# graphdeco-inria/hierarchical-3d-gaussians

Measured on NVIDIA H100. Metric: train-step images/sec (fwd+bwd) @1080p, 3M Gaussians, SH-3, higher is better.
Workload: dtype f32

## Files before the change

### hierarchical-3d-gaussians_b200/csrc/preprocess_backward.cu

```cuda
#include "common.cuh"
#include "cov_grad.cuh"

namespace h3dgs {

__device__ __constant__ float bSH_C2[5] = {1.0925484305920792f, -1.0925484305920792f, 0.31539156525252005f,
                                           -1.0925484305920792f, 0.5462742152960396f};
__device__ __constant__ float bSH_C3[7] = {-0.5900435899266435f, 2.890611442640554f, -0.4570457994644658f,
                                           0.3731763325901154f, -0.4570457994644658f, 1.445305721320277f,
                                           -0.5900435899266435f};
constexpr float bSH_C0 = 0.28209479177387814f;
constexpr float bSH_C1 = 0.4886025119029199f;

__device__ __forceinline__ void store_zero(float* p, int n) {
    for (int k = 0; k < n; k++) p[k] = 0.f;
}

__global__ void __launch_bounds__(128)
preprocess_backward_kernel(int row0, int P, const RowCycle cyc, int deg, int M, const float* __restrict__ means3D, const float* __restrict__ scales,
                           float scale_mod, const float* __restrict__ rots, const float* __restrict__ shs,
                           const float* __restrict__ cov3D_precomp, const float* __restrict__ colors_precomp,
                           const float* __restrict__ ts, const int* __restrict__ ridx, const int* __restrict__ pidx,
                           const float* __restrict__ view, const float* __restrict__ proj,
                           const float* __restrict__ campos, int W, int H, float tanx, float tany, float fx, float fy,
                           int use_depth, const int* __restrict__ radii, const uint8_t* __restrict__ rank_mask, const StagePtrs peers,
                           const Record* __restrict__ records,
                           const float* __restrict__ accum, float* __restrict__ dL_dmeans3D,
                           float* __restrict__ dL_dmeans2D, float* __restrict__ dL_dsh, float* __restrict__ dL_dcolors,
                           float* __restrict__ dL_dopacities, float* __restrict__ dL_dscales,
                           float* __restrict__ dL_drots, float* __restrict__ dL_dcov3D)
{
    __shared__ float s_view[16], s_proj[16];
    if (threadIdx.x < 16) { s_view[threadIdx.x] = view[threadIdx.x]; s_proj[threadIdx.x] = proj[threadIdx.x]; }
    __syncthreads();
    const int local = blockIdx.x * blockDim.x + threadIdx.x;
    const int i = cyc.world > 1 ? cyclic_row(cyc, local) : row0 + local;
    if (i >= P) return;

    if (radii[i] <= 0) {
        store_zero(dL_dmeans2D + 3 * i, 3);
        if (ridx) return;
        store_zero(dL_dmeans3D + 3 * i, 3);
        dL_dopacities[i] = 0.f;
        if (dL_dcolors) store_zero(dL_dcolors + 3 * i, 3);
        if (dL_dscales) store_zero(dL_dscales + 3 * i, 3);
        if (dL_drots) store_zero(dL_drots + 4 * i, 4);
        if (dL_dcov3D) store_zero(dL_dcov3D + 6 * i, 6);
        return;
    }

    const float* v = s_view;
    float ac[kAccum];
    if (peers.n > 1) gather_accum_pairs<5>(peers, rank_mask[i], i, 0, ac);
    else {
        const float2* row = reinterpret_cast<const float2*>(accum + (size_t)i * kAccum);
#pragma unroll
        for (int k = 0; k < 5; k++) { const float2 v = row[k]; ac[2 * k] = v.x; ac[2 * k + 1] = v.y; }
    }
    const float g_mx = ac[0] * (0.5f * W), g_my = ac[1] * (0.5f * H);
    const float dcx = -0.5f * ac[2], dcy = -0.5f * ac[3], dcz = -0.5f * ac[4], g_op = ac[5];
    const float g_r = ac[6], g_g = ac[7], g_b = ac[8], g_iv = ac[9];
    int c = i, p = i;
    float t = 1.0f, u = 0.0f;
    if (ridx) {
        c = ridx[i]; p = pidx[i]; if (p < 0) p = c;
        t = ts[i]; u = 1.0f - t;
    }
    const bool lerp = ridx != nullptr && u != 0.0f;
#define LERP(a, b) (lerp ? __fadd_rn(__fmul_rn(t, (a)), __fmul_rn(u, (b))) : (a))
    const float mx = LERP(means3D[3 * c], means3D[3 * p]);
    const float my = LERP(means3D[3 * c + 1], means3D[3 * p + 1]);
    const float mz = LERP(means3D[3 * c + 2], means3D[3 * p + 2]);
    float qsign = 1.0f;

    float cov6[6], R[3][3], Mm[3][3], sc[3], qv[4] = {1.f, 0.f, 0.f, 0.f};
    const bool have_sr = cov3D_precomp == nullptr;
    if (!have_sr) {
#pragma unroll
        for (int k = 0; k < 6; k++) cov6[k] = cov3D_precomp[6 * c + k];
    } else {
        float4 qq = *reinterpret_cast<const float4*>(rots + 4 * c);
        if (lerp) {
            float4 qp = *reinterpret_cast<const float4*>(rots + 4 * p);
            const float dot = __fadd_rn(__fadd_rn(__fadd_rn(__fmul_rn(qq.x, qp.x), __fmul_rn(qq.y, qp.y)), __fmul_rn(qq.z, qp.z)), __fmul_rn(qq.w, qp.w));
            if (dot < 0.f) qsign = -1.0f;
            qq.x = LERP(qq.x, qsign * qp.x); qq.y = LERP(qq.y, qsign * qp.y);
            qq.z = LERP(qq.z, qsign * qp.z); qq.w = LERP(qq.w, qsign * qp.w);
        }
        qv[0] = qq.x; qv[1] = qq.y; qv[2] = qq.z; qv[3] = qq.w;
#pragma unroll
        for (int k = 0; k < 3; k++) sc[k] = scale_mod * LERP(scales[3 * c + k], scales[3 * p + k]);
        cov3d_from_scale_quat(sc, qv, R, Mm, cov6);
    }

    CovGradOut cg;
    cov_chain_backward(v, mx, my, mz, fx, fy, tanx, tany, kFovClamp, kDilation, cov6, dcx, dcy, dcz, g_iv, use_depth != 0,
                       have_sr, sc, qv, R, Mm, scale_mod, cg);
    float dmean[3] = {cg.dmean[0], cg.dmean[1], cg.dmean[2]};
    {
        const float* q = s_proj;
        const float hw = q[3] * mx + q[7] * my + q[11] * mz + q[15];
        const float m_w = 1.0f / (hw + kWEps);
        const float mul1 = (q[0] * mx + q[4] * my + q[8] * mz + q[12]) * m_w * m_w;
        const float mul2 = (q[1] * mx + q[5] * my + q[9] * mz + q[13]) * m_w * m_w;
        dmean[0] += (q[0] * m_w - q[3] * mul1) * g_mx + (q[1] * m_w - q[3] * mul2) * g_my;
        dmean[1] += (q[4] * m_w - q[7] * mul1) * g_mx + (q[5] * m_w - q[7] * mul2) * g_my;
        dmean[2] += (q[8] * m_w - q[11] * mul1) * g_mx + (q[9] * m_w - q[11] * mul2) * g_my;
    }
    dL_dmeans2D[3 * i] = g_mx; dL_dmeans2D[3 * i + 1] = g_my; dL_dmeans2D[3 * i + 2] = 0.f;
#define EMIT(ptr, width, k, val)                                                           \
    do {                                                                                   \
        const float v__ = (val);                                                           \
        if (!ridx) (ptr)[(size_t)i * (width) + (k)] = v__;                                 \
        else {                                                                             \
            atomicAdd((ptr) + (size_t)c * (width) + (k), t * v__);                         \
            if (lerp) atomicAdd((ptr) + (size_t)p * (width) + (k), u * v__);               \
        }                                                                                  \
    } while (0)
    EMIT(dL_dopacities, 1, 0, g_op);

    if (colors_precomp && dL_dcolors) { dL_dcolors[3 * c] = g_r; dL_dcolors[3 * c + 1] = g_g; dL_dcolors[3 * c + 2] = g_b; }
    EMIT(dL_dmeans3D, 3, 0, dmean[0]); EMIT(dL_dmeans3D, 3, 1, dmean[1]); EMIT(dL_dmeans3D, 3, 2, dmean[2]);

    if (!have_sr) {
        if (dL_dcov3D) {
#pragma unroll
            for (int k = 0; k < 6; k++) dL_dcov3D[6 * c + k] = cg.g6[k];
        }
    } else {
#pragma unroll
        for (int k = 0; k < 3; k++) EMIT(dL_dscales, 3, k, cg.dscale[k]);
        const float4 dq = make_float4(cg.dq[0], cg.dq[1], cg.dq[2], cg.dq[3]);
        if (!ridx) *reinterpret_cast<float4*>(dL_drots + 4 * i) = dq;
        else {
            atomicAdd(reinterpret_cast<float4*>(dL_drots) + c, make_float4(t * dq.x, t * dq.y, t * dq.z, t * dq.w));
            if (lerp) {
                const float us = u * qsign;
                atomicAdd(reinterpret_cast<float4*>(dL_drots) + p, make_float4(us * dq.x, us * dq.y, us * dq.z, us * dq.w));
            }
        }
    }
#undef EMIT
#undef LERP
}

__global__ void __launch_bounds__(128)
sh_backward_kernel(int row0, int P, const RowCycle cyc, int deg, int M, const float* __restrict__ means3D, const float* __restrict__ shs,
                   const float* __restrict__ ts, const int* __restrict__ ridx, const int* __restrict__ pidx,
                   const float* __restrict__ campos, const int* __restrict__ radii, const uint8_t* __restrict__ rank_mask,
                   const StagePtrs peers, const Record* __restrict__ records,
                   const float* __restrict__ accum, float* __restrict__ dL_dmeans3D, float* __restrict__ dL_dsh)
{
    const int local = blockIdx.x * blockDim.x + threadIdx.x;
    const int i = cyc.world > 1 ? cyclic_row(cyc, local) : row0 + local;
    if (i >= P) return;
    const int SH3 = M * 3;
    if (radii[i] <= 0) {
        if (!ridx) {
            float* o = dL_dsh + (size_t)i * SH3;
            if ((SH3 & 3) == 0) { for (int k = 0; k < SH3 / 4; k++) reinterpret_cast<float4*>(o)[k] = make_float4(0, 0, 0, 0); }
            else store_zero(o, SH3);
        }
        return;
    }
    int c = i, p = i;
    float t = 1.0f, u = 0.0f;
    if (ridx) {
        c = ridx[i]; p = pidx[i]; if (p < 0) p = c;
        t = ts[i]; u = 1.0f - t;
    }
    const bool lerp = ridx != nullptr && u != 0.0f;
#define LERP(a, b) (lerp ? __fadd_rn(__fmul_rn(t, (a)), __fmul_rn(u, (b))) : (a))
    const float mx = LERP(means3D[3 * c], means3D[3 * p]);
    const float my = LERP(means3D[3 * c + 1], means3D[3 * p + 1]);
    const float mz = LERP(means3D[3 * c + 2], means3D[3 * p + 2]);
    float col[4];
    if (peers.n > 1) gather_accum_pairs<2>(peers, rank_mask[i], i, 3, col);
    else { const float* ac = accum + (size_t)i * kAccum; col[0] = ac[6]; col[1] = ac[7]; col[2] = ac[8]; }
    const uint32_t kb = __float_as_uint(records[i].b.w);
    const float dRGB[3] = {(kb >> kClampShift) & 1u ? 0.f : col[0], (kb >> (kClampShift + 1)) & 1u ? 0.f : col[1],
                           (kb >> (kClampShift + 2)) & 1u ? 0.f : col[2]};
    const float d0x = mx - campos[0], d0y = my - campos[1], d0z = mz - campos[2];
    const float len = sqrtf(d0x * d0x + d0y * d0y + d0z * d0z);
    const float x = d0x / len, y = d0y / len, z = d0z / len;
    const int ncoef = (deg + 1) * (deg + 1);
    float B[16], Bx[16], By[16], Bz[16];
#pragma unroll
    for (int k = 0; k < 16; k++) { B[k] = 0.f; Bx[k] = 0.f; By[k] = 0.f; Bz[k] = 0.f; }
    B[0] = bSH_C0;
    if (deg > 0) {
        B[1] = -bSH_C1 * y; B[2] = bSH_C1 * z; B[3] = -bSH_C1 * x;
        By[1] = -bSH_C1; Bz[2] = bSH_C1; Bx[3] = -bSH_C1;
        if (deg > 1) {
            const float xx = x * x, yy = y * y, zz = z * z, xy = x * y, yz = y * z, xz = x * z;
            B[4] = bSH_C2[0] * xy; B[5] = bSH_C2[1] * yz; B[6] = bSH_C2[2] * (2.f * zz - xx - yy);
            B[7] = bSH_C2[3] * xz; B[8] = bSH_C2[4] * (xx - yy);
            Bx[4] = bSH_C2[0] * y; By[4] = bSH_C2[0] * x;
            By[5] = bSH_C2[1] * z; Bz[5] = bSH_C2[1] * y;
            Bx[6] = bSH_C2[2] * 2.f * -x; By[6] = bSH_C2[2] * 2.f * -y; Bz[6] = bSH_C2[2] * 2.f * 2.f * z;
            Bx[7] = bSH_C2[3] * z; Bz[7] = bSH_C2[3] * x;
            Bx[8] = bSH_C2[4] * 2.f * x; By[8] = bSH_C2[4] * 2.f * -y;
            if (deg > 2) {
                B[9] = bSH_C3[0] * y * (3.f * xx - yy); B[10] = bSH_C3[1] * xy * z;
                B[11] = bSH_C3[2] * y * (4.f * zz - xx - yy); B[12] = bSH_C3[3] * z * (2.f * zz - 3.f * xx - 3.f * yy);
                B[13] = bSH_C3[4] * x * (4.f * zz - xx - yy); B[14] = bSH_C3[5] * z * (xx - yy);
                B[15] = bSH_C3[6] * x * (xx - 3.f * yy);
                Bx[9] = bSH_C3[0] * 3.f * 2.f * xy;   By[9] = bSH_C3[0] * 3.f * (xx - yy);
                Bx[10] = bSH_C3[1] * yz;              By[10] = bSH_C3[1] * xz;               Bz[10] = bSH_C3[1] * xy;
                Bx[11] = bSH_C3[2] * -2.f * xy;       By[11] = bSH_C3[2] * (-3.f * yy + 4.f * zz - xx); Bz[11] = bSH_C3[2] * 4.f * 2.f * yz;
                Bx[12] = bSH_C3[3] * -3.f * 2.f * xz; By[12] = bSH_C3[3] * -3.f * 2.f * yz;  Bz[12] = bSH_C3[3] * 3.f * (2.f * zz - xx - yy);
                Bx[13] = bSH_C3[4] * (-3.f * xx + 4.f * zz - yy); By[13] = bSH_C3[4] * -2.f * xy; Bz[13] = bSH_C3[4] * 4.f * 2.f * xz;
                Bx[14] = bSH_C3[5] * 2.f * xz;        By[14] = bSH_C3[5] * -2.f * yz;        Bz[14] = bSH_C3[5] * (xx - yy);
                Bx[15] = bSH_C3[6] * 3.f * (xx - yy); By[15] = bSH_C3[6] * -3.f * 2.f * xy;
            }
        }
    }
    float ddx = 0.f, ddy = 0.f, ddz = 0.f;
    const float* shc = shs + (size_t)c * SH3;
    const float* shp = shs + (size_t)p * SH3;
    float* dshi = dL_dsh + (size_t)i * SH3;
    if ((SH3 & 3) == 0) {
#pragma unroll
        for (int q = 0; q < 12; q++) {
            if (4 * q < SH3) {
                float o4[4] = {0.f, 0.f, 0.f, 0.f};
                if (4 * q < 3 * ncoef) {
                    float4 v = __ldg(reinterpret_cast<const float4*>(shc) + q);
                    if (lerp) {
                        const float4 w = __ldg(reinterpret_cast<const float4*>(shp) + q);
                        v.x = LERP(v.x, w.x); v.y = LERP(v.y, w.y); v.z = LERP(v.z, w.z); v.w = LERP(v.w, w.w);
                    }
                    const float sv[4] = {v.x, v.y, v.z, v.w};
#pragma unroll
                    for (int r = 0; r < 4; r++) {
                        const int e = 4 * q + r, k = e / 3, ch = e - 3 * k;
                        const float g = dRGB[ch];
                        o4[r] = B[k] * g;
                        ddx += Bx[k] * sv[r] * g; ddy += By[k] * sv[r] * g; ddz += Bz[k] * sv[r] * g;
                    }
                }
                if (!ridx) reinterpret_cast<float4*>(dshi)[q] = make_float4(o4[0], o4[1], o4[2], o4[3]);
                else if (4 * q < 3 * ncoef) {
                    atomicAdd(reinterpret_cast<float4*>(dL_dsh + (size_t)c * SH3) + q, make_float4(t * o4[0], t * o4[1], t * o4[2], t * o4[3]));
                    if (lerp) atomicAdd(reinterpret_cast<float4*>(dL_dsh + (size_t)p * SH3) + q, make_float4(u * o4[0], u * o4[1], u * o4[2], u * o4[3]));
                }
            }
        }
    } else {
#pragma unroll
        for (int e = 0; e < 48; e++) {
            if (e < SH3) {
                const int k = e / 3, ch = e - 3 * k;
                float o = 0.f;
                if (e < 3 * ncoef) {
                    const float sv = LERP(__ldg(shc + e), __ldg(shp + e));
                    const float g = dRGB[ch];
                    o = B[k] * g;
                    ddx += Bx[k] * sv * g; ddy += By[k] * sv * g; ddz += Bz[k] * sv * g;
                }
                if (!ridx) dshi[e] = o;
                else if (e < 3 * ncoef) {
                    atomicAdd(dL_dsh + (size_t)c * SH3 + e, t * o);
                    if (lerp) atomicAdd(dL_dsh + (size_t)p * SH3 + e, u * o);
                }
            }
        }
    }
    const float sum2 = d0x * d0x + d0y * d0y + d0z * d0z;
    const float invsum32 = 1.0f / sqrtf(sum2 * sum2 * sum2);
    const float dm0 = ((sum2 - d0x * d0x) * ddx - d0y * d0x * ddy - d0z * d0x * ddz) * invsum32;
    const float dm1 = (-d0x * d0y * ddx + (sum2 - d0y * d0y) * ddy - d0z * d0y * ddz) * invsum32;
    const float dm2 = (-d0x * d0z * ddx - d0y * d0z * ddy + (sum2 - d0z * d0z) * ddz) * invsum32;
    if (!ridx) {
        dL_dmeans3D[3 * i] += dm0; dL_dmeans3D[3 * i + 1] += dm1; dL_dmeans3D[3 * i + 2] += dm2;
    } else {
        atomicAdd(dL_dmeans3D + 3 * (size_t)c + 0, t * dm0); atomicAdd(dL_dmeans3D + 3 * (size_t)c + 1, t * dm1);
        atomicAdd(dL_dmeans3D + 3 * (size_t)c + 2, t * dm2);
        if (lerp) {
            atomicAdd(dL_dmeans3D + 3 * (size_t)p + 0, u * dm0); atomicAdd(dL_dmeans3D + 3 * (size_t)p + 1, u * dm1);
            atomicAdd(dL_dmeans3D + 3 * (size_t)p + 2, u * dm2);
        }
    }
#undef LERP
}

__global__ void __launch_bounds__(256)
peer_push_kernel(int P, const RowCycle cyc, const uint8_t* __restrict__ rank_mask, const float* __restrict__ accum,
                 const PeerPtrs stages)
{
    const int i = blockIdx.x * blockDim.x + threadIdx.x;
    if (i >= P) return;
    if (!((rank_mask[i] >> cyc.rank) & 1u)) return;
    const int owner = (i >> cyc.shift) % cyc.world;
    if (owner == cyc.rank) return;
    float* dst = nullptr;
#pragma unroll
    for (int r = 0; r < H3DGS_MAX_PEERS; r++) if (r == owner) dst = static_cast<float*>(stages.p[r]);
    float2* d2 = reinterpret_cast<float2*>(dst + ((size_t)cyc.rank * P + i) * kAccum);
    const float2* s2 = reinterpret_cast<const float2*>(accum + (size_t)i * kAccum);
#pragma unroll
    for (int k = 0; k < kAccum / 2; k++) d2[k] = s2[k];
}

int launch_peer_push(const h3dgs_raster_args& a, const uint8_t* rank_mask, const float* accum, cudaStream_t s)
{
    if (a.P == 0 || a.peer_count <= 1) return H3DGS_OK;
    const RowCycle cyc = row_cycle(a);
    peer_push_kernel<<<(a.P + 255) / 256, 256, 0, s>>>(a.P, cyc, rank_mask, accum, peer_ptrs(a.peer_stage, a.peer_count));
    H3_LAUNCHED("peer_push", a.debug, s);
    return H3DGS_OK;
}

int launch_preprocess_backward(const h3dgs_raster_args& a, const int32_t* radii, const uint8_t* rank_mask, const Record* records,
                               const float* accum, float* dL_dmeans3D, float* dL_dmeans2D, float* dL_dsh,
                               float* dL_dcolors, float* dL_dopacities, float* dL_dscales, float* dL_drots,
                               float* dL_dcov3D, cudaStream_t s)
{
    if (a.P == 0) return H3DGS_OK;
    const float fx = a.image_width / (2.0f * a.tanfovx), fy = a.image_height / (2.0f * a.tanfovy);
    const RowCycle cyc = row_cycle(a);
    const int r0 = (cyc.world > 1 || a.grad_row_end <= a.grad_row_begin) ? 0 : a.grad_row_begin;
    const int r1 = (cyc.world > 1 || a.grad_row_end <= a.grad_row_begin) ? a.P : min(a.grad_row_end, a.P);
    const int rows = cyc.world > 1 ? cyclic_local_rows(cyc, a.P) : r1 - r0;
    if (rows <= 0) return H3DGS_OK;
    ProfScope prof(H3DGS_STAGE_PREPROCESS_BWD, s);
    preprocess_backward_kernel<<<(rows + 127) / 128, 128, 0, s>>>(
        r0, r1, cyc, a.sh_degree, a.sh_coeffs, a.means3D, a.scales, a.scale_modifier, a.rotations, a.shs, a.cov3D_precomp,
        a.colors_precomp, a.interpolation_weights, a.render_indices, a.parent_indices, a.viewmatrix, a.projmatrix, a.campos, a.image_width, a.image_height, a.tanfovx, a.tanfovy,
        fx, fy, a.do_depth, radii, rank_mask, stage_ptrs(a, accum), records, accum, dL_dmeans3D, dL_dmeans2D, dL_dsh, dL_dcolors, dL_dopacities,
        dL_dscales, dL_drots, dL_dcov3D);
    H3_LAUNCHED("preprocess_backward", a.debug, s);
    return H3DGS_OK;
}

int launch_sh_backward(const h3dgs_raster_args& a, const int32_t* radii, const uint8_t* rank_mask, const Record* records,
                       const float* accum, float* dL_dmeans3D, float* dL_dsh, cudaStream_t s)
{
    if (a.P == 0 || a.colors_precomp) return H3DGS_OK;
    const RowCycle cyc = row_cycle(a);
    const int r0 = (cyc.world > 1 || a.grad_row_end <= a.grad_row_begin) ? 0 : a.grad_row_begin;
    const int r1 = (cyc.world > 1 || a.grad_row_end <= a.grad_row_begin) ? a.P : min(a.grad_row_end, a.P);
    const int rows = cyc.world > 1 ? cyclic_local_rows(cyc, a.P) : r1 - r0;
    if (rows <= 0) return H3DGS_OK;
    ProfScope prof(H3DGS_STAGE_SH_BACKWARD, s);
    sh_backward_kernel<<<(rows + 127) / 128, 128, 0, s>>>(r0, r1, cyc, a.sh_degree, a.sh_coeffs, a.means3D, a.shs,
                                                         a.interpolation_weights, a.render_indices, a.parent_indices,
                                                         a.campos, radii, rank_mask, stage_ptrs(a, accum), records, accum,
                                                         dL_dmeans3D, dL_dsh);
    H3_LAUNCHED("sh_backward", a.debug, s);
    return H3DGS_OK;
}

}
```

Baseline: 317.9.

## Stage SH rows through shared memory for coalesced loads and stores in SH backward

Adds a templated SH backward kernel in which each warp cooperatively loads the SH coefficient rows of its 32 Gaussians into padded shared memory with coalesced float4 reads, computes per-thread gradients from shared memory, then writes dL_dsh back cooperatively. This replaces the per-thread strided 192-byte row accesses, which coalesce poorly, and factors the SH basis computation into a shared helper. The cost is about 26KB of shared memory per 128-thread block at degree 3, which may limit occupancy.

```diff
diff --git a/hierarchical-3d-gaussians_b200/csrc/preprocess_backward.cu b/hierarchical-3d-gaussians_b200/csrc/preprocess_backward.cu
--- a/hierarchical-3d-gaussians_b200/csrc/preprocess_backward.cu
+++ b/hierarchical-3d-gaussians_b200/csrc/preprocess_backward.cu
@@ -143,47 +143,9 @@
 #undef LERP
 }
 
-__global__ void __launch_bounds__(128)
-sh_backward_kernel(int row0, int P, const RowCycle cyc, int deg, int M, const float* __restrict__ means3D, const float* __restrict__ shs,
-                   const float* __restrict__ ts, const int* __restrict__ ridx, const int* __restrict__ pidx,
-                   const float* __restrict__ campos, const int* __restrict__ radii, const uint8_t* __restrict__ rank_mask,
-                   const StagePtrs peers, const Record* __restrict__ records,
-                   const float* __restrict__ accum, float* __restrict__ dL_dmeans3D, float* __restrict__ dL_dsh)
-{
-    const int local = blockIdx.x * blockDim.x + threadIdx.x;
-    const int i = cyc.world > 1 ? cyclic_row(cyc, local) : row0 + local;
-    if (i >= P) return;
-    const int SH3 = M * 3;
-    if (radii[i] <= 0) {
-        if (!ridx) {
-            float* o = dL_dsh + (size_t)i * SH3;
-            if ((SH3 & 3) == 0) { for (int k = 0; k < SH3 / 4; k++) reinterpret_cast<float4*>(o)[k] = make_float4(0, 0, 0, 0); }
-            else store_zero(o, SH3);
-        }
-        return;
-    }
-    int c = i, p = i;
-    float t = 1.0f, u = 0.0f;
-    if (ridx) {
-        c = ridx[i]; p = pidx[i]; if (p < 0) p = c;
-        t = ts[i]; u = 1.0f - t;
-    }
-    const bool lerp = ridx != nullptr && u != 0.0f;
-#define LERP(a, b) (lerp ? __fadd_rn(__fmul_rn(t, (a)), __fmul_rn(u, (b))) : (a))
-    const float mx = LERP(means3D[3 * c], means3D[3 * p]);
-    const float my = LERP(means3D[3 * c + 1], means3D[3 * p + 1]);
-    const float mz = LERP(means3D[3 * c + 2], means3D[3 * p + 2]);
-    float col[4];
-    if (peers.n > 1) gather_accum_pairs<2>(peers, rank_mask[i], i, 3, col);
-    else { const float* ac = accum + (size_t)i * kAccum; col[0] = ac[6]; col[1] = ac[7]; col[2] = ac[8]; }
-    const uint32_t kb = __float_as_uint(records[i].b.w);
-    const float dRGB[3] = {(kb >> kClampShift) & 1u ? 0.f : col[0], (kb >> (kClampShift + 1)) & 1u ? 0.f : col[1],
-                           (kb >> (kClampShift + 2)) & 1u ? 0.f : col[2]};
-    const float d0x = mx - campos[0], d0y = my - campos[1], d0z = mz - campos[2];
-    const float len = sqrtf(d0x * d0x + d0y * d0y + d0z * d0z);
-    const float x = d0x / len, y = d0y / len, z = d0z / len;
-    const int ncoef = (deg + 1) * (deg + 1);
-    float B[16], Bx[16], By[16], Bz[16];
+__device__ __forceinline__ void sh_basis(int deg, float x, float y, float z, float (&B)[16], float (&Bx)[16], float (&By)[16],
+                                         float (&Bz)[16])
+{
 #pragma unroll
     for (int k = 0; k < 16; k++) { B[k] = 0.f; Bx[k] = 0.f; By[k] = 0.f; Bz[k] = 0.f; }
     B[0] = bSH_C0;
@@ -214,6 +176,50 @@
             }
         }
     }
+}
+
+__global__ void __launch_bounds__(128)
+sh_backward_kernel(int row0, int P, const RowCycle cyc, int deg, int M, const float* __restrict__ means3D, const float* __restrict__ shs,
+                   const float* __restrict__ ts, const int* __restrict__ ridx, const int* __restrict__ pidx,
+                   const float* __restrict__ campos, const int* __restrict__ radii, const uint8_t* __restrict__ rank_mask,
+                   const StagePtrs peers, const Record* __restrict__ records,
+                   const float* __restrict__ accum, float* __restrict__ dL_dmeans3D, float* __restrict__ dL_dsh)
+{
+    const int local = blockIdx.x * blockDim.x + threadIdx.x;
+    const int i = cyc.world > 1 ? cyclic_row(cyc, local) : row0 + local;
+    if (i >= P) return;
+    const int SH3 = M * 3;
+    if (radii[i] <= 0) {
+        if (!ridx) {
+            float* o = dL_dsh + (size_t)i * SH3;
+            if ((SH3 & 3) == 0) { for (int k = 0; k < SH3 / 4; k++) reinterpret_cast<float4*>(o)[k] = make_float4(0, 0, 0, 0); }
+            else store_zero(o, SH3);
+        }
+        return;
+    }
+    int c = i, p = i;
+    float t = 1.0f, u = 0.0f;
+    if (ridx) {
+        c = ridx[i]; p = pidx[i]; if (p < 0) p = c;
+        t = ts[i]; u = 1.0f - t;
+    }
+    const bool lerp = ridx != nullptr && u != 0.0f;
+#define LERP(a, b) (lerp ? __fadd_rn(__fmul_rn(t, (a)), __fmul_rn(u, (b))) : (a))
+    const float mx = LERP(means3D[3 * c], means3D[3 * p]);
+    const float my = LERP(means3D[3 * c + 1], means3D[3 * p + 1]);
+    const float mz = LERP(means3D[3 * c + 2], means3D[3 * p + 2]);
+    float col[4];
+    if (peers.n > 1) gather_accum_pairs<2>(peers, rank_mask[i], i, 3, col);
+    else { const float* ac = accum + (size_t)i * kAccum; col[0] = ac[6]; col[1] = ac[7]; col[2] = ac[8]; }
+    const uint32_t kb = __float_as_uint(records[i].b.w);
+    const float dRGB[3] = {(kb >> kClampShift) & 1u ? 0.f : col[0], (kb >> (kClampShift + 1)) & 1u ? 0.f : col[1],
+                           (kb >> (kClampShift + 2)) & 1u ? 0.f : col[2]};
+    const float d0x = mx - campos[0], d0y = my - campos[1], d0z = mz - campos[2];
+    const float len = sqrtf(d0x * d0x + d0y * d0y + d0z * d0z);
+    const float x = d0x / len, y = d0y / len, z = d0z / len;
+    const int ncoef = (deg + 1) * (deg + 1);
+    float B[16], Bx[16], By[16], Bz[16];
+    sh_basis(deg, x, y, z, B, Bx, By, Bz);
     float ddx = 0.f, ddy = 0.f, ddz = 0.f;
     const float* shc = shs + (size_t)c * SH3;
     const float* shp = shs + (size_t)p * SH3;
@@ -283,6 +289,121 @@
 #undef LERP
 }
 
+template <int Q>
+__global__ void __launch_bounds__(128)
+sh_backward_rows_kernel(int row0, int P, const RowCycle cyc, int deg, const float* __restrict__ means3D, const float* __restrict__ shs,
+                        const float* __restrict__ ts, const int* __restrict__ ridx, const int* __restrict__ pidx,
+                        const float* __restrict__ campos, const int* __restrict__ radii, const uint8_t* __restrict__ rank_mask,
+                        const StagePtrs peers, const Record* __restrict__ records,
+                        const float* __restrict__ accum, float* __restrict__ dL_dmeans3D, float* __restrict__ dL_dsh)
+{
+    constexpr int SH3 = 4 * Q;
+    constexpr int kStride = SH3 + 4;
+    __shared__ __align__(16) float s_row[128 * kStride];
+    __shared__ int s_c[128], s_p[128];
+    __shared__ float s_t[128], s_u[128];
+    const int tid = threadIdx.x, lane = tid & 31, wb = tid - lane;
+    const int local = blockIdx.x * blockDim.x + threadIdx.x;
+    const int i = cyc.world > 1 ? cyclic_row(cyc, local) : row0 + local;
+    const bool live = i < P && radii[i] > 0;
+    int c = i, p = i;
+    float t = 1.0f, u = 0.0f;
+    if (live && ridx) {
+        c = ridx[i]; p = pidx[i]; if (p < 0) p = c;
+        t = ts[i]; u = 1.0f - t;
+    }
+    const bool lerp = live && ridx != nullptr && u != 0.0f;
+    if (i < P && !live && !ridx) {
+#pragma unroll
+        for (int q = 0; q < Q; q++) reinterpret_cast<float4*>(dL_dsh + (size_t)i * SH3)[q] = make_float4(0.f, 0.f, 0.f, 0.f);
+    }
+    s_c[tid] = live ? c : -1; s_p[tid] = lerp ? p : -1; s_t[tid] = t; s_u[tid] = u;
+    __syncwarp();
+    for (int k = lane; k < 32 * Q; k += 32) {
+        const int r = wb + k / Q, q = k % Q;
+        const int cr = s_c[r];
+        if (cr < 0) continue;
+        float4 v = __ldg(reinterpret_cast<const float4*>(shs + (size_t)cr * SH3) + q);
+        const int pr = s_p[r];
+        if (pr >= 0) {
+            const float4 w = __ldg(reinterpret_cast<const float4*>(shs + (size_t)pr * SH3) + q);
+            const float tr = s_t[r], ur = s_u[r];
+            v.x = __fadd_rn(__fmul_rn(tr, v.x), __fmul_rn(ur, w.x)); v.y = __fadd_rn(__fmul_rn(tr, v.y), __fmul_rn(ur, w.y));
+            v.z = __fadd_rn(__fmul_rn(tr, v.z), __fmul_rn(ur, w.z)); v.w = __fadd_rn(__fmul_rn(tr, v.w), __fmul_rn(ur, w.w));
+        }
+        reinterpret_cast<float4*>(s_row + r * kStride)[q] = v;
+    }
+    __syncwarp();
+    const int ncoef = (deg + 1) * (deg + 1);
+    if (live) {
+#define LERP(a, b) (lerp ? __fadd_rn(__fmul_rn(t, (a)), __fmul_rn(u, (b))) : (a))
+        const float mx = LERP(means3D[3 * c], means3D[3 * p]);
+        const float my = LERP(means3D[3 * c + 1], means3D[3 * p + 1]);
+        const float mz = LERP(means3D[3 * c + 2], means3D[3 * p + 2]);
+#undef LERP
+        float col[4];
+        if (peers.n > 1) gather_accum_pairs<2>(peers, rank_mask[i], i, 3, col);
+        else { const float* ac = accum + (size_t)i * kAccum; col[0] = ac[6]; col[1] = ac[7]; col[2] = ac[8]; }
+        const uint32_t kb = __float_as_uint(records[i].b.w);
+        const float dRGB[3] = {(kb >> kClampShift) & 1u ? 0.f : col[0], (kb >> (kClampShift + 1)) & 1u ? 0.f : col[1],
+                               (kb >> (kClampShift + 2)) & 1u ? 0.f : col[2]};
+        const float d0x = mx - campos[0], d0y = my - campos[1], d0z = mz - campos[2];
+        const float len = sqrtf(d0x * d0x + d0y * d0y + d0z * d0z);
+        const float x = d0x / len, y = d0y / len, z = d0z / len;
+        float B[16], Bx[16], By[16], Bz[16];
+        sh_basis(deg, x, y, z, B, Bx, By, Bz);
+        float ddx = 0.f, ddy = 0.f, ddz = 0.f;
+        float4* slot = reinterpret_cast<float4*>(s_row + tid * kStride);
+#pragma unroll
+        for (int q = 0; q < Q; q++) {
+            float o4[4] = {0.f, 0.f, 0.f, 0.f};
+            if (4 * q < 3 * ncoef) {
+                const float4 v = slot[q];
+                const float sv[4] = {v.x, v.y, v.z, v.w};
+#pragma unroll
+                for (int r = 0; r < 4; r++) {
+                    const int e = 4 * q + r, k = e / 3, ch = e - 3 * k;
+                    const float g = dRGB[ch];
+                    o4[r] = B[k] * g;
+                    ddx += Bx[k] * sv[r] * g; ddy += By[k] * sv[r] * g; ddz += Bz[k] * sv[r] * g;
+                }
+            }
+            slot[q] = make_float4(o4[0], o4[1], o4[2], o4[3]);
+        }
+        const float sum2 = d0x * d0x + d0y * d0y + d0z * d0z;
+        const float invsum32 = 1.0f / sqrtf(sum2 * sum2 * sum2);
+        const float dm0 = ((sum2 - d0x * d0x) * ddx - d0y * d0x * ddy - d0z * d0x * ddz) * invsum32;
+        const float dm1 = (-d0x * d0y * ddx + (sum2 - d0y * d0y) * ddy - d0z * d0y * ddz) * invsum32;
+        const float dm2 = (-d0x * d0z * ddx - d0y * d0z * ddy + (sum2 - d0z * d0z) * ddz) * invsum32;
+        if (!ridx) {
+            dL_dmeans3D[3 * i] += dm0; dL_dmeans3D[3 * i + 1] += dm1; dL_dmeans3D[3 * i + 2] += dm2;
+        } else {
+            atomicAdd(dL_dmeans3D + 3 * (size_t)c + 0, t * dm0); atomicAdd(dL_dmeans3D + 3 * (size_t)c + 1, t * dm1);
+            atomicAdd(dL_dmeans3D + 3 * (size_t)c + 2, t * dm2);
+            if (lerp) {
+                atomicAdd(dL_dmeans3D + 3 * (size_t)p + 0, u * dm0); atomicAdd(dL_dmeans3D + 3 * (size_t)p + 1, u * dm1);
+                atomicAdd(dL_dmeans3D + 3 * (size_t)p + 2, u * dm2);
+            }
+        }
+    }
+    __syncwarp();
+    for (int k = lane; k < 32 * Q; k += 32) {
+        const int r = wb + k / Q, q = k % Q;
+        const int cr = s_c[r];
+        if (cr < 0) continue;
+        const float4 o = reinterpret_cast<const float4*>(s_row + r * kStride)[q];
+        if (!ridx) { reinterpret_cast<float4*>(dL_dsh + (size_t)cr * SH3)[q] = o; continue; }
+        if (4 * q >= 3 * ncoef) continue;
+        const float tr = s_t[r];
+        atomicAdd(reinterpret_cast<float4*>(dL_dsh + (size_t)cr * SH3) + q, make_float4(tr * o.x, tr * o.y, tr * o.z, tr * o.w));
+        const int pr = s_p[r];
+        if (pr >= 0) {
+            const float ur = s_u[r];
+            atomicAdd(reinterpret_cast<float4*>(dL_dsh + (size_t)pr * SH3) + q, make_float4(ur * o.x, ur * o.y, ur * o.z, ur * o.w));
+        }
+    }
+}
+
 __global__ void __launch_bounds__(256)
 peer_push_kernel(int P, const RowCycle cyc, const uint8_t* __restrict__ rank_mask, const float* __restrict__ accum,
                  const PeerPtrs stages)
@@ -342,6 +463,15 @@
     const int rows = cyc.world > 1 ? cyclic_local_rows(cyc, a.P) : r1 - r0;
     if (rows <= 0) return H3DGS_OK;
     ProfScope prof(H3DGS_STAGE_SH_BACKWARD, s);
+    if ((a.sh_coeffs & 3) == 0) {
+        auto kernel = a.sh_coeffs == 16 ? sh_backward_rows_kernel<12> : a.sh_coeffs == 12 ? sh_backward_rows_kernel<9>
+                    : a.sh_coeffs == 8 ? sh_backward_rows_kernel<6> : sh_backward_rows_kernel<3>;
+        kernel<<<(rows + 127) / 128, 128, 0, s>>>(r0, r1, cyc, a.sh_degree, a.means3D, a.shs, a.interpolation_weights,
+                                                  a.render_indices, a.parent_indices, a.campos, radii, rank_mask,
+                                                  stage_ptrs(a, accum), records, accum, dL_dmeans3D, dL_dsh);
+        H3_LAUNCHED("sh_backward", a.debug, s);
+        return H3DGS_OK;
+    }
     sh_backward_kernel<<<(rows + 127) / 128, 128, 0, s>>>(r0, r1, cyc, a.sh_degree, a.sh_coeffs, a.means3D, a.shs,
                                                          a.interpolation_weights, a.render_indices, a.parent_indices,
                                                          a.campos, radii, rank_mask, stage_ptrs(a, accum), records, accum,
```

After: 332.6, median of 6. 1.05x the previous value.
